# trvon/yams

Hardware: AMD Instinct MI355X
Metric: k-NN QPS + recall@k, 100M x 768 fp32 cosine top-100; ingest GB/s SHA-256+CDC (higher is better)
Workload: dtype i8 (MFMA filter, exact i32 accumulate) + f64 (exact re-score)

## Files before the change

yams_amd/csrc/accel_ctx.cpp:

```cpp
#include "accel_ctx.h"

#include <algorithm>
#include <array>
#include <atomic>
#include <condition_variable>
#include <cstdlib>
#include <cstring>
#include <map>
#include <memory>
#include <mutex>
#include <sstream>
#include <thread>

namespace yams_accel {

yams_status_t fail(yams_accel_ctx* ctx, yams_status_t st, const std::string& msg) {
    if (ctx) ctx->last_error = msg;
    return st;
}

yams_status_t hip_fail(yams_accel_ctx* ctx, hipError_t e, const char* what) {
    std::string m = std::string("HIP error ") + hipGetErrorName(e) + " (" + hipGetErrorString(e) +
                    ") in " + what;
    (void)hipGetLastError();
// ... 77 lines not shown
    for (const BigBuf& b : drop) {
        (void)hipSetDevice(b.device);
        if (hipFree(b.p) != hipSuccess) (void)hipGetLastError();
        freed += b.cap;
    }
    (void)hipSetDevice(before);
    return freed;
}

yams_status_t ws_get(yams_accel_ctx* ctx, const char* name, size_t bytes, void** out) {
    auto& b = ctx->ws_ns.empty() ? ctx->bufs[name] : ctx->bufs[ctx->ws_ns + name];
    if (bytes == 0) bytes = 16;
    if (b.cap < bytes) {
        if (b.p) {
            YA_HIP(ctx, hipStreamSynchronize(ctx->stream));
            YA_HIP(ctx, hipFree(b.p));
            b.p = nullptr; b.cap = 0;
        }
        size_t want = bytes + bytes / 8;
        want = (want + 255) & ~static_cast<size_t>(255);
        hipError_t e = ya_malloc(&b.p, want);
        if (e != hipSuccess) {
            b.p = nullptr;
            return hip_fail(ctx, e, (std::string("hipMalloc workspace '") + name + "' of " +
                                     std::to_string(want) + " bytes").c_str());
        }
        b.cap = want;
    }
    *out = b.p;
    return YAMS_OK;
}

size_t ws_trim(yams_accel_ctx* ctx, size_t keep_bytes) {
    size_t freed = 0;
    bool synced = false;
    for (auto& kv : ctx->bufs) {
        auto& b = kv.second;
        if (!b.p || b.cap <= keep_bytes) continue;
        if (!synced) { (void)hipStreamSynchronize(ctx->stream); synced = true; }
        if (hipFree(b.p) != hipSuccess) (void)hipGetLastError();
        freed += b.cap;
        b.p = nullptr; b.cap = 0;
    }
    return freed;
}

yams_status_t pinned_get(yams_accel_ctx* ctx, size_t bytes, void** out) {
    if (ctx->pinned_cap < bytes) {
        if (ctx->pinned) {
            YA_HIP(ctx, hipStreamSynchronize(ctx->stream));
            YA_HIP(ctx, hipHostFree(ctx->pinned));
            ctx->pinned = nullptr; ctx->pinned_cap = 0;
        }
        size_t want = (bytes * 2 + 4095) & ~static_cast<size_t>(4095);
        YA_HIP(ctx, ya_host_malloc(&ctx->pinned, want, hipHostMallocDefault));
        ctx->pinned_cap = want;
// ... 279 lines not shown
    YA_HIP(ctx, hipGetDeviceProperties(&p, ctx->device));
    size_t free_b = 0, total_b = 0;
    (void)hipMemGetInfo(&free_b, &total_b);
    std::ostringstream os;
    os << "{\"backend\":\"hip\",\"arch\":\"" << p.gcnArchName << "\",\"name\":\"" << p.name
       << "\",\"compute_units\":" << p.multiProcessorCount << ",\"clock_khz\":" << p.clockRate
       << ",\"memory_clock_khz\":" << p.memoryClockRate << ",\"memory_bus_bits\":" << p.memoryBusWidth
       << ",\"hbm_bytes\":" << total_b << ",\"hbm_free_bytes\":" << free_b
       << ",\"lds_per_block\":" << p.sharedMemPerBlock << ",\"wavefront\":" << p.warpSize
       << ",\"l2_bytes\":" << p.l2CacheSize << ",\"version\":\"" << YAMS_ACCEL_VERSION_STRING << "\"";
    const auto& hi = ctx->host_ingest;
    if (hi.batches)
        os << ",\"last_host_ingest\":{\"bytes\":" << hi.bytes << ",\"batches\":" << hi.batches << ",\"batch_bytes\":" << hi.batch_bytes
           << ",\"slots\":" << hi.slots << ",\"alloc_ms\":" << hi.alloc_ms
           << ",\"release_ms\":" << hi.release_ms << ",\"total_ms\":" << hi.total_ms << "}";
    os << "}";
    const std::string s = os.str();
    char* buf = static_cast<char*>(std::malloc(s.size() + 1));
    if (!buf) return YAMS_ERR_INTERNAL;
    std::memcpy(buf, s.c_str(), s.size() + 1);
    *out_json = buf;
    return YAMS_OK;
}

void yams_accel_free_string(char* s) { std::free(s); }

uint64_t yams_accel_trim(int device) { return static_cast<uint64_t>(yams_accel::big_trim(device)); }

yams_status_t yams_accel_malloc(yams_accel_ctx* ctx, size_t bytes, void** out_dev) {
    if (!ctx || !out_dev) return YAMS_ERR_INVALID_ARG;
// ... 72 lines not shown
```

yams_amd/csrc/accel_ctx.h:

```cpp
#pragma once
#include <hip/hip_runtime.h>

#include <condition_variable>
#include <cstdint>
#include <functional>
#include <map>
#include <mutex>
#include <string>
#include <vector>

#include "../../include/yams_mi355x_accel.h"

struct yams_accel_gate {
    int device = 0;
    std::mutex mu;
    std::condition_variable cv;
    hipEvent_t last = nullptr;
    bool armed = false;
    yams_accel_ctx* holder = nullptr;
};

struct yams_accel_ctx {
    int device = 0;
    yams_accel_gate* gate = nullptr;
// ... 8 lines not shown
    struct Buf { void* p = nullptr; size_t cap = 0; };
    std::map<std::string, Buf> bufs;
    std::string ws_ns;
    struct TierHint { uint64_t n_rows = 0; bool bf16_first = false; uint32_t served = 0; uint8_t depth[2] = {0, 0}; uint32_t served_deep[2] = {0, 0}; };
    std::map<const void*, TierHint> tier_hints;
    void* pinned = nullptr;
    size_t pinned_cap = 0;

    bool timing = false;
    struct Span { hipEvent_t a, b; };
    std::map<std::string, std::vector<Span>> spans;
    std::vector<hipEvent_t> event_pool;

    struct HostIngestStats { double alloc_ms = 0, release_ms = 0, total_ms = 0; uint64_t batch_bytes = 0, bytes = 0; uint32_t batches = 0, slots = 0; } host_ingest;
    yams_ingest_result_t ingest{};
};

namespace yams_accel {

yams_status_t fail(yams_accel_ctx* ctx, yams_status_t st, const std::string& msg);
yams_status_t hip_fail(yams_accel_ctx* ctx, hipError_t e, const char* what);

yams_status_t ws_get(yams_accel_ctx* ctx, const char* name, size_t bytes, void** out);
size_t ws_trim(yams_accel_ctx* ctx, size_t keep_bytes);
yams_status_t pinned_get(yams_accel_ctx* ctx, size_t bytes, void** out);

hipError_t staged_h2d(void* dst, const void* src, size_t bytes, hipStream_t stream);

struct GatedSweep {
    yams_accel_ctx* ctx; hipStream_t st; std::unique_lock<std::mutex> lk;
// ... 70 lines not shown
```

yams_amd/csrc/scan_api.cpp:

```cpp
#include <chrono>
#include <algorithm>
#include <cmath>
#include <cstdio>
#include <cstdlib>
#include <cstring>
#include <vector>

#include "accel_ctx.h"
#include "scan_launch.h"

using namespace yams_accel;

namespace {

constexpr uint64_t kMfmaMinRows = 4096;
constexpr uint64_t kExactKeyBudget = 1ull << 31;
constexpr size_t kStatWords = 16;

uint32_t round_up(uint32_t v, uint32_t m) { return (v + m - 1) / m * m; }

ScanPlan make_plan(uint64_t n_rows, uint32_t dim, uint32_t nq, uint32_t k, bool bf16, int passes, bool l2_band, int depth = 0) {
    ScanPlan p;
    p.n_rows = n_rows; p.dim = dim; p.n_queries = nq;
    p.tile_rows = bf16 ? 256 : kTileRows;
// ... 468 lines not shown
    YA_TRY(ws_get(ctx, "work32", static_cast<size_t>(2) * nq * std::max(1u, gchunks) * plan.tau_rank * 4, (void**)&f.d_work32));
    const uint32_t lchunks = (plan.list_cap + kSelectCap - 1) / kSelectCap, keep_max = kRescoreMax + 1;
    YA_TRY(ws_get(ctx, "work64", static_cast<size_t>(2) * nq * lchunks * keep_max * 8, (void**)&f.d_work64));
    L.tau = f.d_tau; L.tau_out = f.d_tau; L.list_count = b.d_lcount; L.list = f.d_list;
    if (i8) {
        L.i8_q_form = i8_takes_q_form(L, f.bf16_version);
        if (corpus->row_mask && corpus->row_mask_count) L.i8_mask_inflation = static_cast<double>(corpus->n_rows) / static_cast<double>(corpus->row_mask_count);
        const uint64_t regions = i8_log_regions(L);
        L.log_cap = i8_log_capacity(L);
        YA_TRY(ws_get(ctx, "i8_log_key", static_cast<size_t>(regions) * L.log_cap * i8_log_entry_bytes(L), (void**)&L.log_key));
        YA_TRY(ws_get(ctx, "i8_log_q", static_cast<size_t>(regions) * L.log_cap * 4, (void**)&L.log_q));
        const uint64_t sync_words = i8_sync_words(L);
        const size_t z_cnt = (static_cast<size_t>(regions) * 4 + 255) & ~size_t(255), z_over = (static_cast<size_t>(nq) * 4 + 255) & ~size_t(255);
        unsigned char* zeroed;
        YA_TRY(ws_get(ctx, "i8_zeroed", z_cnt + z_over + static_cast<size_t>(sync_words) * 4, (void**)&zeroed));
        YA_HIP(ctx, launch_prep_i8(st, b.d_qprep, nq, L.q_pad, b.dim, const_cast<int8_t*>(L.q_i8), const_cast<float*>(L.q_meta), L.i8_l2,
                                   reinterpret_cast<uint32_t*>(zeroed), (z_cnt + z_over) / 4 + sync_words, (corpus->i8_flags & YAMS_SCAN_I8_ROTATED) != 0));
        L.log_cnt = reinterpret_cast<uint32_t*>(zeroed);
        L.q_over = f.d_qover = reinterpret_cast<uint32_t*>(zeroed + z_cnt);
        if (sync_words) L.i8_sync = reinterpret_cast<uint32_t*>(zeroed + z_cnt + z_over);
    }
    { TimedRegion tr(ctx, "scan_sample");
      if (i8) YA_HIP(ctx, launch_scan_i8(st, L, 0, f.bf16_version));
      else if (bf16) YA_HIP(ctx, launch_scan_bf16(st, L, b.metric, 0, f.passes, f.bf16_version)); else YA_HIP(ctx, launch_scan_sample(st, L, b.metric));
      tr.end(); }
    if (b.retry) YA_HIP(ctx, hipMemcpyAsync(f.d_tau, b.retry->forced_tau, static_cast<size_t>(nq) * 4, hipMemcpyDeviceToDevice, st));
    else YA_HIP(ctx, launch_select_tau(st, L, f.d_work32));
    if (i8 && L.i8_l2) {
        YA_HIP(ctx, launch_i8_l2_thresholds(st, f.d_tau, L.q_meta, nq, L.q_pad, b.dim, b.d_l2_stats, const_cast<float*>(L.q_thr), const_cast<uint32_t*>(L.i8_q_bias)));
        YA_HIP(ctx, launch_i8_l2_rows(st, corpus->rows_nsq, corpus->rows_i8_meta, b.d_l2_nmin, corpus->n_rows, b.d_l2_stats, const_cast<float*>(L.i8_l2_meta),
                                      const_cast<uint8_t*>(L.i8_row_bias)));
    } else if (i8) YA_HIP(ctx, launch_i8_thresholds(st, f.d_tau, L.q_meta, nq, L.q_pad, const_cast<float*>(L.q_thr)));
    if (i8) YA_HIP(ctx, launch_i8_collect_sample(st, L)); else YA_HIP(ctx, launch_collect_sample(st, L));
    if (i8 && L.i8_l2) YA_HIP(ctx, launch_i8_l2_add_special(st, L, b.d_l2_special, b.l2_n_special));
    { GatedSweep gs(ctx, st);
      TimedRegion tr(ctx, "scan_filter");
      if (i8) YA_HIP(ctx, launch_scan_i8(st, L, 1, f.bf16_version));
      else if (bf16) YA_HIP(ctx, launch_scan_bf16(st, L, b.metric, 1, f.passes, f.bf16_version)); else YA_HIP(ctx, launch_scan_filter(st, L, b.metric));
      tr.end();
      gs.leave(); }
    if (i8) YA_HIP(ctx, launch_i8_log_gather(st, L));
#ifdef YAMS_ACCEL_MEASURE
    if (i8 && L.i8_sync) if (const char* dump = std::getenv("YAMS_ACCEL_DUMP_SYNC")) {
        std::vector<uint32_t> h(i8_sync_words(L));
        YA_HIP(ctx, hipMemcpyAsync(h.data(), L.i8_sync, h.size() * 4, hipMemcpyDeviceToHost, st));
        YA_HIP(ctx, hipStreamSynchronize(st));
        if (FILE* fp = std::fopen(dump, "wb")) { std::fwrite(h.data(), 4, h.size(), fp); std::fclose(fp); }
    }
    const int bv = f.bf16_version;
    if (bv != 2 && bv != 3 && bv != 4 && bv != 20 && bv != 30 && bv != 40 && bv != 50 && bv != 70 && bv != 80 && !(bv >= 81 && bv <= 99)) {
        YA_HIP(ctx, hipStreamSynchronize(st));
        YA_HIP(ctx, hipMemsetAsync(b.io.out_counts, 0, static_cast<size_t>(nq) * 4, st));
        *done = true;
    }
#endif
    return YAMS_OK;
}

yams_status_t rescore(const Batch& b, const Filter& f, uint32_t n_slots, const uint32_t* d_qmap, uint32_t n_cand) {
    const yams_scan_corpus_t* corpus = b.io.corpus;
    const uint64_t* res; uint64_t res_stride;
    YA_HIP(b.ctx, launch_select_lists(b.st, f.d_list, b.d_lcount, f.L.plan.list_cap, n_slots, d_qmap, n_cand + 1, f.d_work64, &res, &res_stride));
// ... 435 lines not shown
```

yams_amd/csrc/scan_args.h:

```cpp
#pragma once
#include "common.h"

namespace yams_accel {

enum { MODE_SAMPLE = 0, MODE_FILTER = 1 };

struct ScanArgs {
    const float* rows;
    const uint16_t* rows_bf16;
    const float* rows_nsq;
    const int8_t* rows_i8;
    const float* rows_i8_meta;
    const int8_t* q_i8;
    const float* q_meta;
    const float* q_thr;
    uint64_t* log_key;
    uint32_t* log_q;
    uint32_t* log_cnt;
    uint32_t log_cap;
    uint32_t* q_over;
    uint32_t* i8_sync;
    const uint8_t* i8_row_bias;
    const uint32_t* i8_q_bias;
    float l2_eps;
    const float* qprep;
    const uint16_t* q_hi;
    const uint16_t* q_lo;
    uint32_t q_pad;
    const uint32_t* row_mask;
    uint64_t n_rows;
    uint32_t dim;
    uint32_t n_queries;
    uint32_t n_sel_tiles;
    uint32_t stride;
    uint32_t n_qtiles;
    float* dense;
// ... 20 lines not shown
```

yams_amd/csrc/scan_i8_kernel.hip:

```cpp
#include <cstdlib>
#include <type_traits>

#include "lds_dma.h"
#include "scan_args.h"

namespace yams_accel {

using i32x4v = __attribute__((ext_vector_type(4))) int;

constexpr int I8_ROWS = 256, I8_QUERIES = 256, I8_THREADS = 512;
constexpr int I8_SLAB = 64;
constexpr int I8_NST = 4;
constexpr int I8_A_BYTES = I8_ROWS * I8_SLAB;
constexpr int I8_B_BYTES = I8_QUERIES * I8_SLAB;
constexpr int I8_STAGE = I8_A_BYTES + I8_B_BYTES;
constexpr int I8_BLOCK_ROWS = 64;

__device__ __forceinline__ int i8_swz(int row) {
    const int j = (row >> 2) & 3;
    return (((j ^ (j >> 1)) & 1) << 1) | (j >> 1);
}

__host__ __device__ __forceinline__ uint64_t i8_blocked_offset(uint64_t row, uint32_t col, uint32_t dim) {
    const uint32_t j = static_cast<uint32_t>(row & 15u), slab = col >> 6, chunk = (col >> 4) & 3u;
// ... 358 lines not shown
static_assert(R_ZS_LOG + 8 * R_ZS_ENTRIES * 12 <= R_LDS, "the survivor buffers must fit the LDS the ring has left");
template <int ABL = 0, bool L2 = false, bool DIRECT = false, int ZSM = 0, bool SAMPLE = false>
__global__ __launch_bounds__(R_THREADS, 1) void scan_tiles_i8r_kernel(ScanArgs a, uint32_t n_units, uint32_t n_qt, uint32_t n_streams, uint32_t window) {
    static_assert(ZSM == 0 || (DIRECT && !L2 && ABL == 0), "the short strip boundary exists for the direct cosine kernel");
    static_assert(!SAMPLE || (DIRECT && !L2 && ABL == 0 && ZSM == 0), "the sample pass exists in the plain direct cosine form");
    static_assert((ZSM & ~(2 | 4 | 64)) == 0, "ZSM bits: 2 thresholds in LDS, 4 survivors in LDS, 64 early boundary");
    constexpr bool ZT = (ZSM & 2) != 0, ZL = (ZSM & 4) != 0;
    constexpr bool EARLY = (ZSM & 64) != 0;
    static_assert(!EARLY || (ZT && ZL), "the early boundary builds on the plain form with its threshold halves and its survivors in LDS");
    const uint32_t pace_mask = (1u << ((window >> 16) & 255u)) - 1u;
    __shared__ __attribute__((aligned(16))) unsigned char lds[R_LDS];

    const uint32_t bid = blockIdx.x;
    const uint32_t xcd = bid & 7u, slot = bid >> 3;
    const uint32_t qt = slot % n_qt, st = slot / n_qt;
    if (st >= (n_streams >> 3)) return;
    const uint32_t stream = st * 8u + xcd;
    if (stream >= n_units) return;

#ifdef YAMS_ACCEL_MEASURE
    const uint64_t t_begin = wall_clock64();
#endif
    const int tid = threadIdx.x;
    const int lane = tid & 63;
    const int wid = __builtin_amdgcn_readfirstlane(tid >> 6);
    const int l15 = lane & 15, lq = lane >> 4;
    const uint32_t dim = a.dim;
    const int nslab = dim / I8_SLAB;
    const uint32_t q0 = qt * R_QUERIES;
    const uint32_t lds0 = static_cast<uint32_t>(reinterpret_cast<uintptr_t>(
        (__attribute__((address_space(3))) unsigned char*)lds));
    const uint32_t ringW = __builtin_amdgcn_readfirstlane(lds0 + R_MAX_SLABS * R_B_SLAB + wid * R_RING);
    const unsigned char* ring = lds + R_MAX_SLABS * R_B_SLAB + wid * R_RING;
    const uint64_t n_blocks = (a.n_rows + I8_BLOCK_ROWS - 1) / I8_BLOCK_ROWS;
    const uint64_t past_end = n_blocks * I8_BLOCK_ROWS;

    struct Geo {
        uint64_t row0;
        const unsigned char* base;
    };
    const uint32_t lane16 = static_cast<uint32_t>(lane) * 16u;
    const uint32_t piece_row_stride = static_cast<uint32_t>(nslab) * 1024u;
    auto unit_of = [&](uint32_t k) __attribute__((always_inline)) -> uint32_t { return stream + (k >> 1) * n_streams; };
    auto locate = [&](uint32_t k, Geo& g) __attribute__((always_inline)) {
        const uint32_t un_ = unit_of(k);
        const uint32_t sel = un_ < n_units ? 2u * un_ + (k & 1u) : 0xffffffffu;
        uint64_t row0 = past_end;
        if (sel < a.n_sel_tiles) {
            const uint32_t tile = SAMPLE ? sel * a.stride : sel + sel / (a.stride - 1u) + 1u;
            row0 = static_cast<uint64_t>(tile) * I8_ROWS + static_cast<uint32_t>((wid & 3) * 64);
        }
        g.row0 = row0;
        const uint64_t rowb = row0 < past_end ? row0 : past_end - 64;
        g.base = reinterpret_cast<const unsigned char*>(a.rows_i8) + (rowb / 16) * piece_row_stride;
    };
    auto piece = [&](const unsigned char* sbase, int ss, int P, int rb) __attribute__((always_inline)) {
        lds_dma16_s(sbase + static_cast<uint32_t>(rb) * piece_row_stride + static_cast<uint32_t>(ss) * 1024u, lane16,
                    ringW + P * 4096 + rb * 1024);
// ... 382 lines not shown
#pragma unroll
            for (int rb = 0; rb < 4; ++rb)
#pragma unroll
                for (int cb = 0; cb < 8; ++cb)
#pragma unroll
                    for (int r = 0; r < 4; ++r) t += acc[rb][cb][r];
            if (t == 123456789 && a.list_cap == 0xffffffffu) a.list_count[0] = 1;
        }
        if (!EARLY && THR && __builtin_amdgcn_ballot_w64(hot != 0) != 0) emit_survivors();
        if (!more) break;
        cur = nxt;
        k_cur = k_nxt; k_nxt = k_fut; k_fut = k_new;
    }
    if (ZL) zs_flush();
    if (__builtin_amdgcn_mbcnt_hi(~0u, __builtin_amdgcn_mbcnt_lo(~0u, 0u)) == 0u && ABL == 0 && !SAMPLE) a.log_cnt[log_region] = log_pos < a.log_cap ? log_pos : a.log_cap;
    asm volatile("s_waitcnt vmcnt(0)" ::: "memory");
#ifdef YAMS_ACCEL_MEASURE
    if (lane == 0 && n_qt <= 8) {
        uint32_t* const dbg = a.i8_sync + (static_cast<uint64_t>(n_streams) * 4u + static_cast<uint64_t>(stream) * 8u + static_cast<uint32_t>(wid)) * 32u;
        dbg[8 + qt] = static_cast<uint32_t>(t_begin);
        dbg[16 + qt] = static_cast<uint32_t>(wall_clock64());
        dbg[24 + qt] = units_read;
    }
#endif
}



#include "scan_i8d_kernel.h"

// ... 310 lines not shown
        const float e = meta[2 * b + 1];
        if (e > 0.f) { sum += static_cast<double>(e); ++cnt; }
    }
    ssum[threadIdx.x] = sum; scnt[threadIdx.x] = cnt;
    __syncthreads();
    for (int st = 128; st >= 1; st >>= 1) {
        if (static_cast<int>(threadIdx.x) < st) { ssum[threadIdx.x] += ssum[threadIdx.x + st]; scnt[threadIdx.x] += scnt[threadIdx.x + st]; }
        __syncthreads();
    }
    if (threadIdx.x == 0 && scnt[0]) {
        atomicAdd(stats, ssum[0]);
        atomicAdd(reinterpret_cast<unsigned long long*>(stats) + 1, static_cast<unsigned long long>(scnt[0]));
    }
}

__global__ __launch_bounds__(256) void prep_i8_kernel(const float* qprep, uint32_t nq, uint32_t q_pad, uint32_t dim,
                                                      int8_t* q_i8, float* q_meta, int raw, uint32_t* zero_words, uint32_t n_zero_words,
                                                      uint32_t rot_p, float rot_scale) {
    const uint32_t q = blockIdx.x;
    for (uint32_t i = q * 256u + threadIdx.x; i < n_zero_words; i += gridDim.x * 256u) zero_words[i] = 0u;
    __shared__ float red[256];
    extern __shared__ float qrot[];
    const bool live = q < nq;
    const float* src = qprep + static_cast<uint64_t>(q) * dim;
    if (rot_p) {
        for (uint32_t i = threadIdx.x; i < dim; i += 256) qrot[i] = live ? __uint_as_float(__float_as_uint(src[i]) ^ rot_sign(i, 1)) : 0.f;
        __syncthreads();
        for (int win = 0; win < 2; ++win) {
            if (win == 1 && rot_p >= dim) break;
            float* w = qrot + (win ? dim - rot_p : 0u);
            if (win) {
                for (uint32_t i = threadIdx.x; i < rot_p; i += 256) w[i] = __uint_as_float(__float_as_uint(w[i]) ^ rot_sign(dim - rot_p + i, 2));
                __syncthreads();
            }
// ... 259 lines not shown
            if (!attr) { (void)hipFuncSetAttribute(reinterpret_cast<const void*>(&shadow_build_i8_kernel<64>), hipFuncAttributeMaxDynamicSharedMemorySize, 65536); attr = true; }
            YA_BUILD_I8(64); break;
        }
        default: return hipErrorInvalidValue;
    }
#undef YA_BUILD_I8
    if (stats && !dry) {
        uint32_t g = static_cast<uint32_t>((n_blocks + 255) / 256);
        if (g > 256) g = 256;
        hipLaunchKernelGGL(i8_meta_stats_kernel, dim3(g), dim3(256), 0, st, out_meta, first_block, first_block + n_blocks, stats);
    }
    return hipGetLastError();
}

hipError_t launch_prep_i8(hipStream_t st, const float* qprep, uint32_t nq, uint32_t q_pad, uint32_t dim,
                          int8_t* q_i8, float* q_meta, bool raw_queries, uint32_t* zero_words, uint64_t n_zero_words, bool rotated) {
    if (q_pad == 0) return hipSuccess;
    if (n_zero_words >> 32) return hipErrorInvalidValue;
    const uint32_t p = rotated ? i8_rotation_window(dim) : 0;
    if (rotated && !p) return hipErrorInvalidValue;
    hipLaunchKernelGGL(prep_i8_kernel, dim3(q_pad), dim3(256), p ? static_cast<size_t>(dim) * 4 : 0, st, qprep, nq, q_pad, dim, q_i8, q_meta, raw_queries ? 1 : 0,
                       zero_words, zero_words ? static_cast<uint32_t>(n_zero_words) : 0u, p, p ? i8_rotation_scale(p) : 0.f);
    return hipGetLastError();
}

float i8_l2_eps(uint32_t dim) { return (static_cast<float>(dim) + 64.f) * 5.9604645e-8f; }

uint32_t i8_l2_max_special() { return I8_L2_MAX_SPECIAL; }

hipError_t launch_i8_l2_add_special(hipStream_t st, const ScanLaunch& L, const uint32_t* special, uint32_t n_special) {
    if (n_special == 0 || L.plan.n_queries == 0) return hipSuccess;
    hipLaunchKernelGGL(i8_l2_add_special_kernel, dim3(L.plan.n_queries), dim3(64), 0, st, special, n_special, L.row_mask,
                       L.plan.n_queries, L.list_count, L.list, L.plan.list_cap);
    return hipGetLastError();
}

hipError_t launch_i8_l2_norm_stats(hipStream_t st, const float* rows_nsq, const float* rows_i8_meta, uint64_t n_rows,
// ... 81 lines not shown

hipError_t launch_i8_collect_sample(hipStream_t st, const ScanLaunch& L) {
    if (L.plan.sample_rows == 0 || L.plan.n_groups == 0) return hipSuccess;
    uint32_t gx = (L.plan.n_groups + 255) / 256;
    if (gx > 64) gx = 64;
#ifdef YAMS_ACCEL_MEASURE
    if (const char* e = std::getenv("YAMS_ACCEL_COLLECT_GX")) { const uint32_t v = static_cast<uint32_t>(std::atoi(e)); if (v >= 1 && v < gx) gx = v; }
#endif
    hipLaunchKernelGGL(i8_collect_sample_kernel, dim3(gx, L.plan.n_queries), dim3(256), 0, st, L.gmax, L.plan.n_groups,
                       L.plan.n_queries, L.rows_i8, L.rows_i8_meta, L.q_i8, L.q_meta, L.q_pad, L.plan.dim, L.plan.sample_stride,
                       L.plan.n_rows, L.row_mask, L.tau, L.list_count, L.list, L.plan.list_cap,
                       L.i8_l2 ? L.rows_nsq : nullptr, L.l2_eps);
    return hipGetLastError();
}

uint64_t i8_sync_words(const ScanLaunch& L) {
    const ResidentPlan r = i8_resident_plan(L);
    return r.use ? static_cast<uint64_t>(r.n_streams) * 12u * 32u * 2u : 0u;
}

uint32_t i8_log_capacity(const ScanLaunch& L) {
    const ScanPlan& p = L.plan;
    const ResidentPlan r = i8_resident_plan(L);
    if (r.use && L.i8_q_form) {
        const double total = static_cast<double>(p.n_queries) * p.tau_rank * p.sample_stride * (L.i8_mask_inflation < 8.0 ? L.i8_mask_inflation : 8.0);
        const double share = total / (static_cast<double>(r.n_streams) * r.n_qt * 4.0);
        const double cap = 4.0 * share + 512.0;
        const uint64_t c = static_cast<uint64_t>(cap < 1.0e6 ? cap : 1.0e6);
        return static_cast<uint32_t>((c + 15) / 16 * 16);
    }
// ... 41 lines not shown
        hipLaunchKernelGGL((i8_log_gather_kernel<false>), dim3(static_cast<uint32_t>((regions + 255) / 256)), dim3(256), 0, st,
                           L.log_key, L.log_q, L.log_cnt, L.log_cap, regions, L.rows_i8_meta, L.q_meta, L.q_thr, L.list_count, L.list,
                           L.plan.list_cap, l2);
    return hipGetLastError();
}

static bool i8r_direct_rows(uint32_t dim, uint32_t n_qt, bool l2) { (void)dim; return l2 ? n_qt >= 4 : true; }

hipError_t launch_scan_i8(hipStream_t st, const ScanLaunch& L, int mode, int version) {
    (void)version;
    ScanArgs a = make_scan_args(L);
    a.n_sel_tiles = mode == MODE_SAMPLE ? L.plan.n_sample_tiles : L.plan.n_filter_tiles;
    if (a.n_sel_tiles == 0) return hipSuccess;
    const uint32_t hgrid = ((2u * a.n_sel_tiles + 7) / 8) * a.n_qtiles * 8;
    const ResidentPlan rp = i8_resident_plan(L);
    if (mode == MODE_SAMPLE) {
        const uint32_t s_units = (L.plan.n_sample_tiles + 1u) / 2u;
        bool resident_sample = rp.use && !L.i8_l2 && L.i8_sync && L.plan.sample_stride >= 2 && !L.i8_sample_small_grid &&
                               (L.i8_form == 2 ? s_units >= 1u : s_units >= 4u * rp.n_streams);
#ifdef YAMS_ACCEL_MEASURE
        if (const char* sv = std::getenv("YAMS_ACCEL_I8R_SAMPLE")) resident_sample = resident_sample && std::atoi(sv) != 0;
        if (version != 2 && version != 3 && version != 0) resident_sample = false;
#endif
        if (resident_sample) {
            a.i8_sync = L.i8_sync + i8_sync_words(L) / 2u;
            hipLaunchKernelGGL((scan_tiles_i8r_kernel<0, false, true, 0, true>), dim3(rp.grid), dim3(R_THREADS), 0, st, a, s_units, rp.n_qt, rp.n_streams, 1u);
        } else if (L.i8_l2) hipLaunchKernelGGL((scan_tiles_i8h_kernel<MODE_SAMPLE, 0, YAMS_SCAN_L2>), dim3(hgrid), dim3(H_THREADS), 0, st, a);
        else hipLaunchKernelGGL((scan_tiles_i8h_kernel<MODE_SAMPLE>), dim3(hgrid), dim3(H_THREADS), 0, st, a);
        return hipGetLastError();
    }
// ... 91 lines not shown
```

yams_amd/csrc/scan_i8d_kernel.h:

```cpp
template <int DUMMY = 0>
__global__ __launch_bounds__(R_THREADS, 1) void scan_tiles_i8d_kernel(ScanArgs a, uint32_t n_units, uint32_t n_qt, uint32_t n_streams, uint32_t window) {
    const uint32_t pace_mask = (1u << ((window >> 16) & 255u)) - 1u;
    __shared__ __attribute__((aligned(16))) unsigned char lds[R_LDS];

    const uint32_t bid = blockIdx.x;
    const uint32_t xcd = bid & 7u, slot = bid >> 3;
    const uint32_t qt = slot % n_qt, st = slot / n_qt;
    if (st >= (n_streams >> 3)) return;
    const uint32_t stream = st * 8u + xcd;
    if (stream >= n_units) return;

#ifdef YAMS_ACCEL_MEASURE
    const uint64_t t_begin = wall_clock64();
#endif
    const int tid = threadIdx.x;
    const int lane = tid & 63;
    const int wid = __builtin_amdgcn_readfirstlane(tid >> 6);
    const int l15 = lane & 15, lq = lane >> 4;
    const uint32_t dim = a.dim;
    const int nslab = dim / I8_SLAB;
    const uint32_t q0 = qt * R_QUERIES;
    const uint32_t lds0 = static_cast<uint32_t>(reinterpret_cast<uintptr_t>((__attribute__((address_space(3))) unsigned char*)lds));
    const uint64_t n_blocks = (a.n_rows + I8_BLOCK_ROWS - 1) / I8_BLOCK_ROWS;
    const uint64_t past_end = n_blocks * I8_BLOCK_ROWS;
    const uint32_t piece_row_stride = static_cast<uint32_t>(nslab) * 1024u;

    struct Geo { uint64_t row0; const unsigned char* base; };
    auto unit_of = [&](uint32_t k) __attribute__((always_inline)) -> uint32_t { return stream + (k >> 1) * n_streams; };
    auto locate = [&](uint32_t k, Geo& g) __attribute__((always_inline)) {
        const uint32_t un_ = unit_of(k);
        const uint32_t sel = un_ < n_units ? 2u * un_ + (k & 1u) : 0xffffffffu;
        uint64_t row0 = past_end;
        if (sel < a.n_sel_tiles) {
            const uint32_t tile = sel + sel / (a.stride - 1u) + 1u;
            row0 = static_cast<uint64_t>(tile) * I8_ROWS + static_cast<uint32_t>((wid & 3) * 64);
        }
        g.row0 = row0;
        const uint64_t rowb = row0 < past_end ? row0 : past_end - 64;
        g.base = reinterpret_cast<const unsigned char*>(a.rows_i8) + (rowb / 16) * piece_row_stride;
    };
    typedef float f2_t __attribute__((ext_vector_type(2)));
    auto meta_ptr = [&](uint64_t row0) __attribute__((always_inline)) -> const float* {
        uint64_t blk = row0 / I8_BLOCK_ROWS;
// ... 214 lines not shown
            uint32_t polls = 0;
            for (; polls < R_POLLS; ++polls) {
                if (__builtin_amdgcn_ballot_w64(sib + R_WINDOW < k_new) == 0) break;
                __builtin_amdgcn_s_sleep(8);
                asm volatile("global_load_dword %0, %1, off sc0 sc1\n\ts_waitcnt vmcnt(0)" : "=v"(sib) : "v"(sync_sib) : "memory");
            }
            if (polls == R_POLLS) pacing = false;
        }
        if (!more) break;
        cur = nxt;
        k_cur = k_nxt; k_nxt = k_fut; k_fut = k_new;
    }
    asm volatile("s_waitcnt vmcnt(0)" : "+v"(fa[0][0]), "+v"(fa[0][1]), "+v"(fa[0][2]), "+v"(fa[0][3]), "+v"(fa[1][0]), "+v"(fa[1][1]), "+v"(fa[1][2]),
                 "+v"(fa[1][3]), "+v"(fa[2][0]), "+v"(fa[2][1]), "+v"(fa[2][2]), "+v"(fa[2][3]) :: "memory");
    zs_flush();
    if (__builtin_amdgcn_mbcnt_hi(~0u, __builtin_amdgcn_mbcnt_lo(~0u, 0u)) == 0u) a.log_cnt[log_region] = log_pos < a.log_cap ? log_pos : a.log_cap;
#ifdef YAMS_ACCEL_MEASURE
    if (lane == 0 && n_qt <= 8) {
        uint32_t* const dbg = a.i8_sync + (static_cast<uint64_t>(n_streams) * 4u + static_cast<uint64_t>(stream) * 8u + static_cast<uint32_t>(wid)) * 32u;
        dbg[8 + qt] = static_cast<uint32_t>(t_begin);
        dbg[16 + qt] = static_cast<uint32_t>(wall_clock64());
        dbg[24 + qt] = units_read;
    }
#endif
}
```

yams_amd/csrc/scan_launch.h:

```cpp
#pragma once
#include "common.h"

namespace yams_accel {

struct ScanLaunch {
    ScanPlan plan;
    const float* rows = nullptr;
    const uint16_t* rows_bf16 = nullptr;
    const float* rows_nsq = nullptr;
    const int8_t* rows_i8 = nullptr;
    const float* rows_i8_meta = nullptr;
    const int8_t* q_i8 = nullptr;
    const float* q_meta = nullptr;
    const float* q_thr = nullptr;
    uint64_t* log_key = nullptr; uint32_t* log_q = nullptr; uint32_t* log_cnt = nullptr; uint32_t log_cap = 0;
    uint32_t* q_over = nullptr;
    uint32_t* i8_sync = nullptr;
    bool i8_l2 = false;
    const float* i8_l2_meta = nullptr;
    const uint8_t* i8_row_bias = nullptr;
    const uint32_t* i8_q_bias = nullptr;
    float l2_eps = 0.f;
    bool i8_sample_small_grid = false;
    int i8_form = 0;
    bool i8_q_form = false;
    double i8_mask_inflation = 1.0;
    int sample_layout = 0;
    const uint32_t* row_mask = nullptr;
    const float* qprep = nullptr;
    const uint16_t* q_hi = nullptr;
    const uint16_t* q_lo = nullptr;
    uint32_t q_pad = 0;
// ... 45 lines not shown
    unsigned long long* dbg = nullptr;
};
uint32_t small_scan_max_survivors();
hipError_t launch_small_scan(hipStream_t st, int metric, const SmallScanArgs& a, uint32_t qb);

constexpr uint32_t kRescoreMax = 2047;

hipError_t launch_prep_queries(hipStream_t st, const float* q, uint32_t nq, uint32_t dim,
                               int metric, float* qprep, double* qnorm, float* qnorm_up,
                               uint32_t* qflags, uint32_t* zero_words = nullptr, uint32_t n_zero_words = 0);
hipError_t launch_prep_split(hipStream_t st, const float* qprep, uint32_t nq, uint32_t q_pad, uint32_t dim,
                             uint32_t slab_k, uint16_t* q_hi, uint16_t* q_lo);
inline uint32_t bf16_slab_k(int passes, uint32_t dim) { return (passes == 1 && (dim & 31u) == 0) ? 32u : 16u; }
hipError_t launch_scan_bf16(hipStream_t st, const ScanLaunch& L, int metric, int mode, int passes, int version);
hipError_t launch_scan_i8(hipStream_t st, const ScanLaunch& L, int mode, int version);
hipError_t launch_prep_i8(hipStream_t st, const float* qprep, uint32_t nq, uint32_t q_pad, uint32_t dim,
                          int8_t* q_i8, float* q_meta, bool raw_queries = false, uint32_t* zero_words = nullptr,
                          uint64_t n_zero_words = 0, bool rotated = false);
hipError_t launch_i8_l2_norm_stats(hipStream_t st, const float* rows_nsq, const float* rows_i8_meta, uint64_t n_rows,
                                   float* nmin, uint32_t* stats, uint32_t* special);
uint32_t i8_l2_max_special();
hipError_t launch_i8_l2_add_special(hipStream_t st, const ScanLaunch& L, const uint32_t* special, uint32_t n_special);
hipError_t launch_i8_l2_thresholds(hipStream_t st, const float* tau, const float* q_meta, uint32_t nq, uint32_t q_pad,
                                   uint32_t dim, const uint32_t* stats, float* q_thr, uint32_t* q_bias);
hipError_t launch_i8_l2_rows(hipStream_t st, const float* rows_nsq, const float* rows_i8_meta, const float* nmin,
                             uint64_t n_rows, const uint32_t* stats, float* l2_meta, uint8_t* row_bias);
float i8_l2_eps(uint32_t dim);
hipError_t launch_shadow_build_i8(hipStream_t st, const float* rows, uint64_t first_row, uint64_t n_rows, uint32_t dim,
                                  int8_t* out_i8, float* out_meta, double* stats, bool rotated = false, uint64_t block_stride = 1,
                                  double* dry = nullptr);
uint32_t i8_rotation_window(uint32_t dim);
uint64_t i8_log_regions(const ScanLaunch& L);
uint32_t i8_log_capacity(const ScanLaunch& L);
// ... 57 lines not shown
```

Before: 16810.

## Rebalance i8 resident scan units across XCDs using per-XCD timing feedback

Replaces the fixed round-robin assignment of scan units to streams with per-XCD contiguous unit ranges whose sizes follow weights kept in a device table. Each filter workgroup records begin/end wall-clock ticks. On the next query batch the prep kernel derives per-XCD throughput and moves the weights toward it with damping, clamped to about ±8%. The aim is to cut tail latency when some XCDs finish later than others, at the cost of extra global tick writes, offset loads and a serial update step in the prep kernel.

```diff
diff --git a/yams_amd/csrc/accel_ctx.cpp b/yams_amd/csrc/accel_ctx.cpp
--- a/yams_amd/csrc/accel_ctx.cpp
+++ b/yams_amd/csrc/accel_ctx.cpp
@@ -1,4 +1,5 @@
 #include "accel_ctx.h"
+#include "xcd_deal.h"
 
 #include <algorithm>
 #include <array>
@@ -115,6 +116,7 @@
     if (b.cap < bytes) {
         if (b.p) {
             YA_HIP(ctx, hipStreamSynchronize(ctx->stream));
+            if (b.p == ctx->xcd_deal.table) ctx->xcd_deal.table = nullptr;
             YA_HIP(ctx, hipFree(b.p));
             b.p = nullptr; b.cap = 0;
         }
@@ -141,6 +143,7 @@
         if (!synced) { (void)hipStreamSynchronize(ctx->stream); synced = true; }
         if (hipFree(b.p) != hipSuccess) (void)hipGetLastError();
         freed += b.cap;
+        if (b.p == ctx->xcd_deal.table) ctx->xcd_deal.table = nullptr;
         b.p = nullptr; b.cap = 0;
     }
     return freed;
@@ -450,6 +453,18 @@
         os << ",\"last_host_ingest\":{\"bytes\":" << hi.bytes << ",\"batches\":" << hi.batches << ",\"batch_bytes\":" << hi.batch_bytes
            << ",\"slots\":" << hi.slots << ",\"alloc_ms\":" << hi.alloc_ms
            << ",\"release_ms\":" << hi.release_ms << ",\"total_ms\":" << hi.total_ms << "}";
+    if (ctx->xcd_deal.table) {
+        uint32_t t[yams_accel::XCD_TABLE_TICKS];
+        YA_HIP(ctx, hipMemcpyAsync(t, ctx->xcd_deal.table, sizeof(t), hipMemcpyDeviceToHost, ctx->stream));
+        YA_HIP(ctx, hipStreamSynchronize(ctx->stream));
+        os << ",\"xcd_deal\":{\"streams_per_xcd\":" << ctx->xcd_deal.streams_x << ",\"units\":" << ctx->xcd_deal.n_units_filter << ",\"weights\":[";
+        for (uint32_t x = 0; x < 8; ++x) os << (x ? "," : "") << t[yams_accel::XCD_TABLE_WEIGHTS + x] / 65536.0;
+        os << "],\"off\":[";
+        for (uint32_t x = 0; x <= 8; ++x) os << (x ? "," : "") << t[yams_accel::XCD_TABLE_OFF_FILTER + x];
+        os << "],\"off_sample\":[";
+        for (uint32_t x = 0; x <= 8; ++x) os << (x ? "," : "") << t[yams_accel::XCD_TABLE_OFF_SAMPLE + x];
+        os << "]}";
+    }
     os << "}";
     const std::string s = os.str();
     char* buf = static_cast<char*>(std::malloc(s.size() + 1));
diff --git a/yams_amd/csrc/accel_ctx.h b/yams_amd/csrc/accel_ctx.h
--- a/yams_amd/csrc/accel_ctx.h
+++ b/yams_amd/csrc/accel_ctx.h
@@ -46,6 +46,8 @@
 
     struct HostIngestStats { double alloc_ms = 0, release_ms = 0, total_ms = 0; uint64_t batch_bytes = 0, bytes = 0; uint32_t batches = 0, slots = 0; } host_ingest;
     yams_ingest_result_t ingest{};
+    struct XcdDealState { const void* rows_i8 = nullptr; uint64_t n_rows = 0; uint32_t dim = 0, n_qt = 0, streams_x = 0, n_units_filter = 0,
+                          n_units_sample = 0, l2 = 0, forced = 0; uint32_t* table = nullptr; } xcd_deal;
 };
 
 namespace yams_accel {
diff --git a/yams_amd/csrc/scan_api.cpp b/yams_amd/csrc/scan_api.cpp
--- a/yams_amd/csrc/scan_api.cpp
+++ b/yams_amd/csrc/scan_api.cpp
@@ -506,8 +506,36 @@
         const size_t z_cnt = (static_cast<size_t>(regions) * 4 + 255) & ~size_t(255), z_over = (static_cast<size_t>(nq) * 4 + 255) & ~size_t(255);
         unsigned char* zeroed;
         YA_TRY(ws_get(ctx, "i8_zeroed", z_cnt + z_over + static_cast<size_t>(sync_words) * 4, (void**)&zeroed));
+        XcdDealPrep deal{};
+        uint64_t deal_words = 0;
+        if (i8_xcd_deal_plan(L, &deal, &deal_words)) {
+            YA_TRY(ws_get(ctx, "i8_xcd", static_cast<size_t>(deal_words) * 4, (void**)&L.i8_xcd));
+            auto& k = ctx->xcd_deal;
+            const bool same = k.table == L.i8_xcd && k.rows_i8 == corpus->rows_i8 && k.n_rows == corpus->n_rows && k.dim == b.dim && k.n_qt == deal.n_qt &&
+                              k.streams_x == deal.streams_x && k.n_units_filter == deal.n_units_filter && k.n_units_sample == deal.n_units_sample &&
+                              k.l2 == (L.i8_l2 ? 1u : 0u) && !k.forced;
+            deal.table = L.i8_xcd;
+            deal.mode = same ? XCD_DEAL_FEEDBACK : XCD_DEAL_RESET;
+            k.table = L.i8_xcd; k.rows_i8 = corpus->rows_i8; k.n_rows = corpus->n_rows; k.dim = b.dim; k.n_qt = deal.n_qt; k.streams_x = deal.streams_x;
+            k.n_units_filter = deal.n_units_filter; k.n_units_sample = deal.n_units_sample; k.l2 = L.i8_l2 ? 1u : 0u; k.forced = 0;
+#ifdef YAMS_ACCEL_MEASURE
+            if (const char* wv = std::getenv("YAMS_ACCEL_XCD_WEIGHTS")) {
+                deal.mode = XCD_DEAL_FORCED;
+                for (int x = 0; x < 8; ++x) deal.forced[x] = XCD_DEAL_ONE;
+                const char* p = wv;
+                for (int x = 0; x < 8 && *p; ++x) {
+                    char* end = nullptr;
+                    const double v = std::strtod(p, &end);
+                    if (end == p) break;
+                    deal.forced[x] = static_cast<uint32_t>(std::min(std::max(v, 0.0), 16.0) * XCD_DEAL_ONE + 0.5);
+                    p = *end == ',' ? end + 1 : end;
+                }
+                k.forced = 1;
+            }
+#endif
+        }
         YA_HIP(ctx, launch_prep_i8(st, b.d_qprep, nq, L.q_pad, b.dim, const_cast<int8_t*>(L.q_i8), const_cast<float*>(L.q_meta), L.i8_l2,
-                                   reinterpret_cast<uint32_t*>(zeroed), (z_cnt + z_over) / 4 + sync_words, (corpus->i8_flags & YAMS_SCAN_I8_ROTATED) != 0));
+                                   reinterpret_cast<uint32_t*>(zeroed), (z_cnt + z_over) / 4 + sync_words, (corpus->i8_flags & YAMS_SCAN_I8_ROTATED) != 0, &deal));
         L.log_cnt = reinterpret_cast<uint32_t*>(zeroed);
         L.q_over = f.d_qover = reinterpret_cast<uint32_t*>(zeroed + z_cnt);
         if (sync_words) L.i8_sync = reinterpret_cast<uint32_t*>(zeroed + z_cnt + z_over);
@@ -533,11 +561,19 @@
       gs.leave(); }
     if (i8) YA_HIP(ctx, launch_i8_log_gather(st, L));
 #ifdef YAMS_ACCEL_MEASURE
-    if (i8 && L.i8_sync) if (const char* dump = std::getenv("YAMS_ACCEL_DUMP_SYNC")) {
+    if (!(i8 && L.i8_sync)) {}
+    else if (const char* dump = std::getenv("YAMS_ACCEL_DUMP_SYNC")) {
         std::vector<uint32_t> h(i8_sync_words(L));
         YA_HIP(ctx, hipMemcpyAsync(h.data(), L.i8_sync, h.size() * 4, hipMemcpyDeviceToHost, st));
         YA_HIP(ctx, hipStreamSynchronize(st));
         if (FILE* fp = std::fopen(dump, "wb")) { std::fwrite(h.data(), 4, h.size(), fp); std::fclose(fp); }
+    } else if (const char* log = std::getenv("YAMS_ACCEL_DUMP_SYNC_LOG")) {
+        std::vector<uint32_t> h(4 + i8_sync_words(L));
+        YA_HIP(ctx, hipMemcpyAsync(h.data() + 4, L.i8_sync, (h.size() - 4) * 4, hipMemcpyDeviceToHost, st));
+        YA_HIP(ctx, hipStreamSynchronize(st));
+        h[0] = 0x58434442u; h[1] = static_cast<uint32_t>(reinterpret_cast<uintptr_t>(ctx)); h[2] = static_cast<uint32_t>(h.size() - 4);
+        h[3] = static_cast<uint32_t>(i8_sync_words(L) / (12u * 32u * 2u));
+        if (FILE* fp = std::fopen(log, "ab")) { std::setvbuf(fp, nullptr, _IONBF, 0); std::fwrite(h.data(), 4, h.size(), fp); std::fclose(fp); }
     }
     const int bv = f.bf16_version;
     if (bv != 2 && bv != 3 && bv != 4 && bv != 20 && bv != 30 && bv != 40 && bv != 50 && bv != 70 && bv != 80 && !(bv >= 81 && bv <= 99)) {
diff --git a/yams_amd/csrc/scan_args.h b/yams_amd/csrc/scan_args.h
--- a/yams_amd/csrc/scan_args.h
+++ b/yams_amd/csrc/scan_args.h
@@ -20,6 +20,8 @@
     uint32_t log_cap;
     uint32_t* q_over;
     uint32_t* i8_sync;
+    const uint32_t* xcd_off;
+    uint32_t* xcd_ticks;
     const uint8_t* i8_row_bias;
     const uint32_t* i8_q_bias;
     float l2_eps;
diff --git a/yams_amd/csrc/scan_i8_kernel.hip b/yams_amd/csrc/scan_i8_kernel.hip
--- a/yams_amd/csrc/scan_i8_kernel.hip
+++ b/yams_amd/csrc/scan_i8_kernel.hip
@@ -1,8 +1,10 @@
+#include <climits>
 #include <cstdlib>
 #include <type_traits>
 
 #include "lds_dma.h"
 #include "scan_args.h"
+#include "xcd_deal.h"
 
 namespace yams_accel {
 
@@ -396,9 +398,12 @@
     const uint32_t bid = blockIdx.x;
     const uint32_t xcd = bid & 7u, slot = bid >> 3;
     const uint32_t qt = slot % n_qt, st = slot / n_qt;
-    if (st >= (n_streams >> 3)) return;
+    const uint32_t streams_x = n_streams >> 3;
+    if (st >= streams_x) return;
     const uint32_t stream = st * 8u + xcd;
-    if (stream >= n_units) return;
+    const uint32_t off_lo = a.xcd_off[xcd], off_hi = a.xcd_off[xcd + 1u] < n_units ? a.xcd_off[xcd + 1u] : n_units;
+    if (xcd_deal_unit(off_lo, off_hi, streams_x, st, 0u) >= n_units) return;
+    if (!SAMPLE && a.xcd_ticks && threadIdx.x == 0) a.xcd_ticks[(stream * n_qt + qt) * XCD_TICKS_PER_WG] = static_cast<uint32_t>(wall_clock64()) | 1u;
 
 #ifdef YAMS_ACCEL_MEASURE
     const uint64_t t_begin = wall_clock64();
@@ -423,7 +428,7 @@
     };
     const uint32_t lane16 = static_cast<uint32_t>(lane) * 16u;
     const uint32_t piece_row_stride = static_cast<uint32_t>(nslab) * 1024u;
-    auto unit_of = [&](uint32_t k) __attribute__((always_inline)) -> uint32_t { return stream + (k >> 1) * n_streams; };
+    auto unit_of = [&](uint32_t k) __attribute__((always_inline)) -> uint32_t { return xcd_deal_unit(off_lo, off_hi, streams_x, st, k >> 1); };
     auto locate = [&](uint32_t k, Geo& g) __attribute__((always_inline)) {
         const uint32_t un_ = unit_of(k);
         const uint32_t sel = un_ < n_units ? 2u * un_ + (k & 1u) : 0xffffffffu;
@@ -836,6 +841,8 @@
     }
     if (ZL) zs_flush();
     if (__builtin_amdgcn_mbcnt_hi(~0u, __builtin_amdgcn_mbcnt_lo(~0u, 0u)) == 0u && ABL == 0 && !SAMPLE) a.log_cnt[log_region] = log_pos < a.log_cap ? log_pos : a.log_cap;
+    if (__builtin_amdgcn_mbcnt_hi(~0u, __builtin_amdgcn_mbcnt_lo(~0u, 0u)) == 0u && !SAMPLE && a.xcd_ticks)
+        a.xcd_ticks[(stream * n_qt + qt) * XCD_TICKS_PER_WG + 1u + static_cast<uint32_t>(wid)] = static_cast<uint32_t>(wall_clock64()) | 1u;
     asm volatile("s_waitcnt vmcnt(0)" ::: "memory");
 #ifdef YAMS_ACCEL_MEASURE
     if (lane == 0 && n_qt <= 8) {
@@ -1176,10 +1183,60 @@
     }
 }
 
+__device__ __forceinline__ void xcd_deal_update(const XcdDealPrep& d) {
+    __shared__ int s_end[XCD_DEAL_XCDS];
+    __shared__ int s_begin;
+    __shared__ uint32_t s_missing, s_ref;
+    uint32_t* const w = d.table + XCD_TABLE_WEIGHTS;
+    uint32_t* const off_f = d.table + XCD_TABLE_OFF_FILTER;
+    uint32_t* const ticks = d.table + XCD_TABLE_TICKS;
+    const uint32_t n_wg = d.streams_x * XCD_DEAL_XCDS * d.n_qt;
+    if (threadIdx.x < XCD_DEAL_XCDS) s_end[threadIdx.x] = INT_MIN;
+    if (threadIdx.x == 0) { s_begin = INT_MAX; s_missing = 0u; s_ref = 0u; }
+    __syncthreads();
+    if (d.mode == XCD_DEAL_FEEDBACK)
+        for (uint32_t g = threadIdx.x; g < n_wg; g += blockDim.x) atomicMax(&s_ref, ticks[g * XCD_TICKS_PER_WG]);
+    __syncthreads();
+    if (d.mode == XCD_DEAL_FEEDBACK) {
+        const uint32_t ref = s_ref;
+        for (uint32_t g = threadIdx.x; g < n_wg; g += blockDim.x) {
+            const uint32_t stream = g / d.n_qt, x = stream & 7u, st = stream >> 3;
+            if (xcd_deal_stream_length(off_f[x], off_f[x + 1u], d.streams_x, st) == 0u) continue;
+            const uint32_t b = ticks[g * XCD_TICKS_PER_WG];
+            if (b == 0u) { atomicOr(&s_missing, 1u); continue; }
+            atomicMin(&s_begin, static_cast<int>(b - ref));
+            for (uint32_t wv = 0; wv < 8u; ++wv) {
+                const uint32_t e = ticks[g * XCD_TICKS_PER_WG + 1u + wv];
+                if (e == 0u) atomicOr(&s_missing, 1u); else atomicMax(&s_end[x], static_cast<int>(e - ref));
+            }
+        }
+    }
+    __syncthreads();
+    for (uint32_t i = threadIdx.x; i < n_wg * XCD_TICKS_PER_WG; i += blockDim.x) ticks[i] = 0u;
+    if (threadIdx.x != 0) return;
+    uint32_t wl[XCD_DEAL_XCDS], off[XCD_DEAL_XCDS + 1];
+    for (uint32_t x = 0; x < XCD_DEAL_XCDS; ++x) wl[x] = d.mode == XCD_DEAL_FEEDBACK ? w[x] : (d.mode == XCD_DEAL_FORCED ? d.forced[x] : XCD_DEAL_ONE);
+    if (d.mode == XCD_DEAL_FEEDBACK && s_missing == 0u && s_begin != INT_MAX) {
+        uint32_t n[XCD_DEAL_XCDS];
+        int64_t t[XCD_DEAL_XCDS];
+        for (uint32_t x = 0; x < XCD_DEAL_XCDS; ++x) {
+            n[x] = off_f[x + 1u] - off_f[x];
+            t[x] = s_end[x] == INT_MIN ? 0 : static_cast<int64_t>(s_end[x]) - s_begin;
+        }
+        xcd_deal_feedback(wl, n, t);
+    }
+    for (uint32_t x = 0; x < XCD_DEAL_XCDS; ++x) w[x] = wl[x];
+    xcd_deal_offsets(wl, d.n_units_filter, d.streams_x, off);
+    for (uint32_t x = 0; x <= XCD_DEAL_XCDS; ++x) off_f[x] = off[x];
+    xcd_deal_offsets(wl, d.n_units_sample, d.streams_x, off);
+    for (uint32_t x = 0; x <= XCD_DEAL_XCDS; ++x) d.table[XCD_TABLE_OFF_SAMPLE + x] = off[x];
+}
+
 __global__ __launch_bounds__(256) void prep_i8_kernel(const float* qprep, uint32_t nq, uint32_t q_pad, uint32_t dim,
                                                       int8_t* q_i8, float* q_meta, int raw, uint32_t* zero_words, uint32_t n_zero_words,
-                                                      uint32_t rot_p, float rot_scale) {
+                                                      uint32_t rot_p, float rot_scale, XcdDealPrep deal) {
     const uint32_t q = blockIdx.x;
+    if (deal.table && q == gridDim.x - 1u) xcd_deal_update(deal);
     for (uint32_t i = q * 256u + threadIdx.x; i < n_zero_words; i += gridDim.x * 256u) zero_words[i] = 0u;
     __shared__ float red[256];
     extern __shared__ float qrot[];
@@ -1469,13 +1526,15 @@
 }
 
 hipError_t launch_prep_i8(hipStream_t st, const float* qprep, uint32_t nq, uint32_t q_pad, uint32_t dim,
-                          int8_t* q_i8, float* q_meta, bool raw_queries, uint32_t* zero_words, uint64_t n_zero_words, bool rotated) {
+                          int8_t* q_i8, float* q_meta, bool raw_queries, uint32_t* zero_words, uint64_t n_zero_words, bool rotated, const XcdDealPrep* deal) {
     if (q_pad == 0) return hipSuccess;
+    XcdDealPrep xd{};
+    if (deal && deal->table) xd = *deal;
     if (n_zero_words >> 32) return hipErrorInvalidValue;
     const uint32_t p = rotated ? i8_rotation_window(dim) : 0;
     if (rotated && !p) return hipErrorInvalidValue;
     hipLaunchKernelGGL(prep_i8_kernel, dim3(q_pad), dim3(256), p ? static_cast<size_t>(dim) * 4 : 0, st, qprep, nq, q_pad, dim, q_i8, q_meta, raw_queries ? 1 : 0,
-                       zero_words, zero_words ? static_cast<uint32_t>(n_zero_words) : 0u, p, p ? i8_rotation_scale(p) : 0.f);
+                       zero_words, zero_words ? static_cast<uint32_t>(n_zero_words) : 0u, p, p ? i8_rotation_scale(p) : 0.f, xd);
     return hipGetLastError();
 }
 
@@ -1587,6 +1646,17 @@
     return hipGetLastError();
 }
 
+bool i8_xcd_deal_plan(const ScanLaunch& L, XcdDealPrep* p, uint64_t* table_words) {
+    const ResidentPlan r = i8_resident_plan(L);
+    if (!r.use) return false;
+    p->n_units_filter = r.n_units;
+    p->n_units_sample = (L.plan.n_sample_tiles + 1u) / 2u;
+    p->streams_x = r.n_streams / XCD_DEAL_XCDS;
+    p->n_qt = r.n_qt;
+    *table_words = XCD_TABLE_TICKS + static_cast<uint64_t>(r.n_streams) * r.n_qt * XCD_TICKS_PER_WG;
+    return true;
+}
+
 uint64_t i8_sync_words(const ScanLaunch& L) {
     const ResidentPlan r = i8_resident_plan(L);
     return r.use ? static_cast<uint64_t>(r.n_streams) * 12u * 32u * 2u : 0u;
@@ -1658,6 +1728,11 @@
     if (a.n_sel_tiles == 0) return hipSuccess;
     const uint32_t hgrid = ((2u * a.n_sel_tiles + 7) / 8) * a.n_qtiles * 8;
     const ResidentPlan rp = i8_resident_plan(L);
+    if (rp.use && !L.i8_xcd) return hipErrorInvalidValue;
+    if (rp.use) {
+        a.xcd_off = L.i8_xcd + (mode == MODE_SAMPLE ? XCD_TABLE_OFF_SAMPLE : XCD_TABLE_OFF_FILTER);
+        a.xcd_ticks = mode == MODE_SAMPLE ? nullptr : L.i8_xcd + XCD_TABLE_TICKS;
+    }
     if (mode == MODE_SAMPLE) {
         const uint32_t s_units = (L.plan.n_sample_tiles + 1u) / 2u;
         bool resident_sample = rp.use && !L.i8_l2 && L.i8_sync && L.plan.sample_stride >= 2 && !L.i8_sample_small_grid &&
diff --git a/yams_amd/csrc/scan_i8d_kernel.h b/yams_amd/csrc/scan_i8d_kernel.h
--- a/yams_amd/csrc/scan_i8d_kernel.h
+++ b/yams_amd/csrc/scan_i8d_kernel.h
@@ -6,12 +6,15 @@
     const uint32_t bid = blockIdx.x;
     const uint32_t xcd = bid & 7u, slot = bid >> 3;
     const uint32_t qt = slot % n_qt, st = slot / n_qt;
-    if (st >= (n_streams >> 3)) return;
+    const uint32_t streams_x = n_streams >> 3;
+    if (st >= streams_x) return;
     const uint32_t stream = st * 8u + xcd;
-    if (stream >= n_units) return;
-
-#ifdef YAMS_ACCEL_MEASURE
-    const uint64_t t_begin = wall_clock64();
+    const uint32_t off_lo = a.xcd_off[xcd], off_hi = a.xcd_off[xcd + 1u] < n_units ? a.xcd_off[xcd + 1u] : n_units;
+    if (xcd_deal_unit(off_lo, off_hi, streams_x, st, 0u) >= n_units) return;
+    if (a.xcd_ticks && threadIdx.x == 0) a.xcd_ticks[(stream * n_qt + qt) * XCD_TICKS_PER_WG] = static_cast<uint32_t>(wall_clock64()) | 1u;
+
+#ifdef YAMS_ACCEL_MEASURE
+    const uint64_t t_begin = wall_clock64(), c_begin = clock64();
 #endif
     const int tid = threadIdx.x;
     const int lane = tid & 63;
@@ -26,7 +29,7 @@
     const uint32_t piece_row_stride = static_cast<uint32_t>(nslab) * 1024u;
 
     struct Geo { uint64_t row0; const unsigned char* base; };
-    auto unit_of = [&](uint32_t k) __attribute__((always_inline)) -> uint32_t { return stream + (k >> 1) * n_streams; };
+    auto unit_of = [&](uint32_t k) __attribute__((always_inline)) -> uint32_t { return xcd_deal_unit(off_lo, off_hi, streams_x, st, k >> 1); };
     auto locate = [&](uint32_t k, Geo& g) __attribute__((always_inline)) {
         const uint32_t un_ = unit_of(k);
         const uint32_t sel = un_ < n_units ? 2u * un_ + (k & 1u) : 0xffffffffu;
@@ -271,13 +274,17 @@
     asm volatile("s_waitcnt vmcnt(0)" : "+v"(fa[0][0]), "+v"(fa[0][1]), "+v"(fa[0][2]), "+v"(fa[0][3]), "+v"(fa[1][0]), "+v"(fa[1][1]), "+v"(fa[1][2]),
                  "+v"(fa[1][3]), "+v"(fa[2][0]), "+v"(fa[2][1]), "+v"(fa[2][2]), "+v"(fa[2][3]) :: "memory");
     zs_flush();
-    if (__builtin_amdgcn_mbcnt_hi(~0u, __builtin_amdgcn_mbcnt_lo(~0u, 0u)) == 0u) a.log_cnt[log_region] = log_pos < a.log_cap ? log_pos : a.log_cap;
+    if (__builtin_amdgcn_mbcnt_hi(~0u, __builtin_amdgcn_mbcnt_lo(~0u, 0u)) == 0u) {
+        a.log_cnt[log_region] = log_pos < a.log_cap ? log_pos : a.log_cap;
+        if (a.xcd_ticks) a.xcd_ticks[(stream * n_qt + qt) * XCD_TICKS_PER_WG + 1u + static_cast<uint32_t>(wid)] = static_cast<uint32_t>(wall_clock64()) | 1u;
+    }
 #ifdef YAMS_ACCEL_MEASURE
     if (lane == 0 && n_qt <= 8) {
         uint32_t* const dbg = a.i8_sync + (static_cast<uint64_t>(n_streams) * 4u + static_cast<uint64_t>(stream) * 8u + static_cast<uint32_t>(wid)) * 32u;
         dbg[8 + qt] = static_cast<uint32_t>(t_begin);
         dbg[16 + qt] = static_cast<uint32_t>(wall_clock64());
         dbg[24 + qt] = units_read;
+        dbg[qt] = static_cast<uint32_t>((clock64() - c_begin) * 100ull / (wall_clock64() - t_begin + 1));
     }
 #endif
 }
diff --git a/yams_amd/csrc/scan_launch.h b/yams_amd/csrc/scan_launch.h
--- a/yams_amd/csrc/scan_launch.h
+++ b/yams_amd/csrc/scan_launch.h
@@ -1,5 +1,6 @@
 #pragma once
 #include "common.h"
+#include "xcd_deal.h"
 
 namespace yams_accel {
 
@@ -16,6 +17,7 @@
     uint64_t* log_key = nullptr; uint32_t* log_q = nullptr; uint32_t* log_cnt = nullptr; uint32_t log_cap = 0;
     uint32_t* q_over = nullptr;
     uint32_t* i8_sync = nullptr;
+    uint32_t* i8_xcd = nullptr;
     bool i8_l2 = false;
     const float* i8_l2_meta = nullptr;
     const uint8_t* i8_row_bias = nullptr;
@@ -91,9 +93,10 @@
 inline uint32_t bf16_slab_k(int passes, uint32_t dim) { return (passes == 1 && (dim & 31u) == 0) ? 32u : 16u; }
 hipError_t launch_scan_bf16(hipStream_t st, const ScanLaunch& L, int metric, int mode, int passes, int version);
 hipError_t launch_scan_i8(hipStream_t st, const ScanLaunch& L, int mode, int version);
+bool i8_xcd_deal_plan(const ScanLaunch& L, XcdDealPrep* p, uint64_t* table_words);
 hipError_t launch_prep_i8(hipStream_t st, const float* qprep, uint32_t nq, uint32_t q_pad, uint32_t dim,
                           int8_t* q_i8, float* q_meta, bool raw_queries = false, uint32_t* zero_words = nullptr,
-                          uint64_t n_zero_words = 0, bool rotated = false);
+                          uint64_t n_zero_words = 0, bool rotated = false, const XcdDealPrep* deal = nullptr);
 hipError_t launch_i8_l2_norm_stats(hipStream_t st, const float* rows_nsq, const float* rows_i8_meta, uint64_t n_rows,
                                    float* nmin, uint32_t* stats, uint32_t* special);
 uint32_t i8_l2_max_special();
diff --git a/yams_amd/csrc/xcd_deal.h b/yams_amd/csrc/xcd_deal.h
--- /dev/null
+++ b/yams_amd/csrc/xcd_deal.h
@@ -0,0 +1,103 @@
+#pragma once
+#include <stdint.h>
+
+#if defined(__HIPCC__) || defined(__CUDACC__)
+#define XCD_DEAL_FN __host__ __device__ inline
+#else
+#define XCD_DEAL_FN inline
+#endif
+
+namespace yams_accel {
+
+constexpr uint32_t XCD_DEAL_XCDS = 8;
+constexpr uint32_t XCD_DEAL_ONE = 65536;
+constexpr int32_t XCD_DEAL_CLAMP = 5242;
+
+XCD_DEAL_FN uint32_t xcd_deal_equal_count(uint32_t n_units, uint32_t streams_x, uint32_t x) {
+    const uint32_t n_streams = streams_x * XCD_DEAL_XCDS;
+    const uint32_t q = n_units / n_streams, r = n_units % n_streams;
+    const uint32_t c = r > x ? (r - x + XCD_DEAL_XCDS - 1) / XCD_DEAL_XCDS : 0u;
+    return q * streams_x + (c < streams_x ? c : streams_x);
+}
+
+XCD_DEAL_FN void xcd_deal_moves(const uint32_t* w, int32_t* e) {
+    uint64_t sum = 0;
+    for (uint32_t x = 0; x < XCD_DEAL_XCDS; ++x) sum += w[x];
+    int64_t pos = 0, neg = 0;
+    for (uint32_t x = 0; x < XCD_DEAL_XCDS; ++x) {
+        int64_t v = sum ? static_cast<int64_t>((static_cast<uint64_t>(w[x]) * XCD_DEAL_XCDS * XCD_DEAL_ONE) / sum) - XCD_DEAL_ONE : 0;
+        v = v > XCD_DEAL_CLAMP ? XCD_DEAL_CLAMP : (v < -XCD_DEAL_CLAMP ? -XCD_DEAL_CLAMP : v);
+        e[x] = static_cast<int32_t>(v);
+        if (v > 0) pos += v; else neg -= v;
+    }
+    for (uint32_t x = 0; x < XCD_DEAL_XCDS; ++x) {
+        if (pos > neg && e[x] > 0) e[x] = static_cast<int32_t>(static_cast<int64_t>(e[x]) * neg / pos);
+        else if (neg > pos && e[x] < 0) e[x] = -static_cast<int32_t>(static_cast<int64_t>(-e[x]) * pos / neg);
+    }
+}
+
+XCD_DEAL_FN void xcd_deal_offsets(const uint32_t* w, uint32_t n_units, uint32_t streams_x, uint32_t* off) {
+    int32_t e[XCD_DEAL_XCDS];
+    xcd_deal_moves(w, e);
+    int64_t cnt[XCD_DEAL_XCDS];
+    int64_t rest = 0;
+    for (uint32_t x = 0; x < XCD_DEAL_XCDS; ++x) {
+        const int64_t d = static_cast<int64_t>(n_units) * e[x] / static_cast<int64_t>(XCD_DEAL_XCDS * XCD_DEAL_ONE);
+        cnt[x] = static_cast<int64_t>(xcd_deal_equal_count(n_units, streams_x, x)) + d;
+        if (cnt[x] < 0) cnt[x] = 0;
+        rest -= cnt[x];
+    }
+    rest += n_units;
+    for (uint32_t x = 0; rest != 0; x = (x + 1) % XCD_DEAL_XCDS) {
+        if (rest > 0) { ++cnt[x]; --rest; }
+        else if (cnt[x] > 0) { --cnt[x]; ++rest; }
+    }
+    off[0] = 0;
+    for (uint32_t x = 0; x < XCD_DEAL_XCDS; ++x) off[x + 1] = off[x] + static_cast<uint32_t>(cnt[x]);
+}
+
+XCD_DEAL_FN uint32_t xcd_deal_unit(uint32_t off_lo, uint32_t off_hi, uint32_t streams_x, uint32_t st, uint32_t j) {
+    const uint64_t u = static_cast<uint64_t>(off_lo) + st + static_cast<uint64_t>(j) * streams_x;
+    return u < off_hi ? static_cast<uint32_t>(u) : 0xffffffffu;
+}
+
+XCD_DEAL_FN uint32_t xcd_deal_stream_length(uint32_t off_lo, uint32_t off_hi, uint32_t streams_x, uint32_t st) {
+    const uint32_t n = off_hi - off_lo;
+    return n > st ? (n - st + streams_x - 1) / streams_x : 0u;
+}
+
+XCD_DEAL_FN uint32_t xcd_deal_max_stream_length(uint32_t n_units, uint32_t streams_x) {
+    const uint32_t n_streams = streams_x * XCD_DEAL_XCDS;
+    const uint64_t xcd_most = static_cast<uint64_t>((n_units + n_streams - 1) / n_streams) * streams_x
+                              + (static_cast<uint64_t>(n_units) * XCD_DEAL_CLAMP) / (XCD_DEAL_XCDS * XCD_DEAL_ONE) + 1u;
+    return static_cast<uint32_t>((xcd_most + streams_x - 1) / streams_x);
+}
+
+XCD_DEAL_FN void xcd_deal_feedback(uint32_t* w, const uint32_t* n, const int64_t* t) {
+    double rate[XCD_DEAL_XCDS], sum = 0.0;
+    for (uint32_t x = 0; x < XCD_DEAL_XCDS; ++x) {
+        if (n[x] == 0 || t[x] <= 0) return;
+        rate[x] = static_cast<double>(n[x]) / static_cast<double>(t[x]);
+        sum += rate[x];
+    }
+    const double lo = static_cast<double>(XCD_DEAL_ONE - XCD_DEAL_CLAMP), hi = static_cast<double>(XCD_DEAL_ONE + XCD_DEAL_CLAMP);
+    for (uint32_t x = 0; x < XCD_DEAL_XCDS; ++x) {
+        double target = rate[x] * XCD_DEAL_XCDS / sum * XCD_DEAL_ONE;
+        target = target < lo ? lo : (target > hi ? hi : target);
+        double v = static_cast<double>(w[x]);
+        v = v < lo ? lo : (v > hi ? hi : v);
+        v += (target - v) * 0.25;
+        w[x] = static_cast<uint32_t>(v + 0.5);
+    }
+}
+
+constexpr uint32_t XCD_TABLE_WEIGHTS = 0;
+constexpr uint32_t XCD_TABLE_OFF_FILTER = 8;
+constexpr uint32_t XCD_TABLE_OFF_SAMPLE = 17;
+constexpr uint32_t XCD_TABLE_TICKS = 32;
+constexpr uint32_t XCD_TICKS_PER_WG = 9;
+
+enum { XCD_DEAL_FEEDBACK = 0, XCD_DEAL_RESET = 1, XCD_DEAL_FORCED = 2 };
+struct XcdDealPrep { uint32_t* table; uint32_t n_units_filter, n_units_sample, streams_x, n_qt, mode; uint32_t forced[8]; };
+
+}
```

Result: faster. 17250 (median of 6 runs) (+2.6%).
